# wbhart/mpir-fft

Measured on AMD Instinct MI355X. Metric: limbs/s for new_mpn_mul N×N-bit at 1/2/4/8 MI355X; % HBM roofline, higher is better.
Workload: dtype u64; 1 GPU; C3: new_mpn_mul depth=15 w=4 n1=n2=20312500 limbs (l=2048 limbs/coeff, NC x NR = 256 x 256, trunc=39936); parallelism=single

## Files before the change

__graft_entry__.py:

```python
import os
import subprocess
import sys

ROOT = os.path.dirname(os.path.abspath(__file__))
CSRC = os.path.join(ROOT, "mpir-fft_amd", "csrc")
LIB = os.path.join(ROOT, "mpir-fft_amd", "libmpfft.so")
HIPCC = os.environ.get("HIPCC", "/opt/rocm/bin/hipcc")


def build_lib(force=False):
    if force:
        subprocess.run(["make", "-s", "-C", CSRC, "clean"], check=True)
    jobs = str(min(8, os.cpu_count() or 1))
    subprocess.run(["make", "-s", "-C", CSRC, "-j" + jobs, "HIPCC=" + HIPCC], check=True)
    subprocess.run(["make", "-s", "-C", CSRC, "-j" + jobs, "HIPCC=" + HIPCC, "pwspill"], check=True)


def build_oracle():
    subprocess.run(["make", "-s", "-C", os.path.join(ROOT, "oracle")], check=True)


def build_c_caller():
    subprocess.run(["make", "-s", "-C", os.path.join(ROOT, "tests", "c_abi")], check=True)


def build_host_tests():
    subprocess.run(["make", "-s", "-C", os.path.join(ROOT, "tests", "pw_host")], check=True)


def build():
    build_lib()
    build_oracle()
    build_c_caller()
    build_host_tests()
    sys.path.insert(0, ROOT)
    import mpfft_loader
    m = mpfft_loader.load()
    assert m.lib().mpfft_version() >= 1


def smoke():
    import numpy as np
    import torch
    sys.path.insert(0, ROOT)
    sys.path.insert(0, os.path.join(ROOT, "oracle"))
    import mpfft_loader
    import oracle as O
    m = mpfft_loader.load()
    assert torch.cuda.is_available(), "smoke() needs a GPU"
    depth, w, n1, n2 = 9, 2, 120, 97
    a = m.fill_random(n1, 0x1001)
    b = m.fill_random(n2, 0x2002)
    dev = torch.device("cuda:0")
    da = torch.from_numpy(a.view(np.int64)).to(dev)
    db = torch.from_numpy(b.view(np.int64)).to(dev)
    dr = torch.zeros(n1 + n2, dtype=torch.int64, device=dev)
    ws = m.alloc_workspace(n1, n2, depth, w, dev)
    m.mul_device(dr, da, n1, db, n2, depth, w, ws)
    torch.cuda.synchronize()
    got = dr.cpu().numpy().view(np.uint64)
    want = O.new_mpn_mul(a, b, depth, w)
    assert (got == want).all(), "GPU new_mpn_mul differs from the oracle"
    assert O.to_int(got) == O.to_int(a) * O.to_int(b), "GPU product is not the exact product"
    r = np.zeros(n1 + n2, dtype=np.uint64)
    m.new_mpn_mul(r, a, n1, b, n2, depth, w)
    assert (r == want).all()
    d6, w6, m1, m2 = 8, 1, 700, 500
    a6 = m.fill_random(m1, 0x61)
    b6 = m.fill_random(m2, 0x62)
    r6 = m.mul6(a6, b6, d6, w6)
    assert (r6 == O.new_mpn_mul6(a6, b6, d6, w6)).all(), "GPU new_mpn_mul6 differs from the oracle"
    assert O.to_int(r6) == O.to_int(a6) * O.to_int(b6)
    print("smoke: ok (depth=%d w=%d n1=%d n2=%d; mul6 depth=%d w=%d n1=%d n2=%d)" % (depth, w, n1, n2, d6, w6, m1, m2))


if __name__ == "__main__":
    build()
    if len(sys.argv) > 1 and sys.argv[1] == "smoke":
        smoke()
```

mpir-fft_amd/csrc/kernels.hpp:

```cpp
#pragma once
#include "coeff.hpp"

struct PassArgs {
    u64 *dig[2];
    u64 *cb[2];
    int *top[2];
    const u64 *src[2];
    long nsrc[2];
    long src_chunk;
    u64 bits1;
    u64 N;
    int l;
    int lbM, lvl0;
    u64 rho;
    long sub_stride, pos_stride;
    int nsub, pos_off;
    int pbb;
    long pbs;
    int sub_off;
    long jNC;
    int zero_from;
    int need;
    int need_lo;
    int tw_mode;
    u64 tw_w;
    int tw_lbR;
    int canon;
    int ngroups;
    int nbuf;
    u64 scale_e;
    int ablate;
    unsigned *zp;
    long zn;
    unsigned long long *dbg;
    int pcarry;
    int pkeep;
    int fill_lo, fill_off;
    u64 fill_rho;
    int fill_hmin;
    int grp0;
};

__device__ inline void pass_clear_flags(const PassArgs &a)
{
    if (!a.zp) return;
    const long nt = (long)blockDim.x * blockDim.y * blockDim.z;
    const long nthr = (long)gridDim.x * gridDim.y * gridDim.z * nt;
    const long bid = ((long)blockIdx.z * gridDim.y + blockIdx.y) * gridDim.x + blockIdx.x;
    const long t = bid * nt + ((long)threadIdx.z * blockDim.y + threadIdx.y) * blockDim.x + threadIdx.x;
    for (long i = t; i < a.zn; i += nthr) a.zp[i] = 0u;
}

struct Lds {
    i64 *stage;
    int *edge;
    u64 *scr;
};

__host__ __device__ inline size_t lds_bytes(int l, int rb, int G, int U, int nw)
{
    size_t st = (size_t)rb * 2 * l * sizeof(i64);
    size_t ed = ((size_t)norm_edge_ints(G, U, nw) * sizeof(int) + 15) / 16 * 16;
    return st + ed + (size_t)norm_scr_u64(G, U, nw) * sizeof(u64);
}

template <int U, int G>
__device__ __forceinline__ Lds lds_carve(unsigned char *smem, int l, int rb, int nw)
{
    Lds d;
    d.stage = (i64 *)smem;
    unsigned char *p = smem + (size_t)rb * 2 * l * sizeof(i64);
    d.edge = (int *)p;
    p += ((size_t)norm_edge_ints(G, U, nw) * sizeof(int) + 15) / 16 * 16;
    d.scr = (u64 *)p;
    return d;
}

template <int U, int G, typename EF>
__device__ __forceinline__ void rotate_all(const WG &c, i64 (&x)[G][2 * U], EF efn, u64 N, int l, i64 *stage,
                                           int rb)
{
    if (U == 1 || rb >= G) {
        bool any = false;
#pragma unroll
        for (int i = 0; i < G; ++i) {
            const u64 e = efn(i);
            if (e) {
                rot_write<U>(c, x[i], stage + (size_t)i * 2 * l, l);
                any = true;
            }
        }
        if (!any) return;
        __syncthreads();
#pragma unroll
        for (int i = 0; i < G; ++i) {
            const u64 e = efn(i);
            if (e) rot_read<U>(c, x[i], stage + (size_t)i * 2 * l, make_rot(e, N), l);
        }
        __syncthreads();
    } else if (U != 1) {
#pragma unroll
        for (int i = 0; i < G; ++i) {
            const u64 e = efn(i);
            if (!e) continue;
// ... 967 lines not shown
```

mpir-fft_amd/csrc/mpfft.hip:

```cpp
#include <hip/hip_runtime.h>
#include <stdint.h>
#include <stdio.h>
#include <stdlib.h>
#include <string.h>
#include <mutex>
#include <string>
#include <vector>

#include "kernels.hpp"
#include "combine.hpp"
#include "fold.hpp"
#include "wdispatch.hpp"
#include "bdispatch.hpp"
#include "pdispatch.hpp"
#include "rdispatch.hpp"
#include "../../include/mpfft.h"

static const char *diag_env(const char *name)
{
#ifdef MPFFT_DIAG
    return getenv(name);
#else
    (void)name;
    return nullptr;
// ... 551 lines not shown
        HIPCHK(hipMemcpyAsync(h, d, nwg * 64, hipMemcpyDeviceToHost, s));
        HIPCHK(hipStreamSynchronize(s));
        double sum[8] = {0};
        long cnt = 0;
        unsigned long long t0 = ~0ull, t1 = 0;
        for (size_t w = 0; w < nwg; ++w) {
            const unsigned long long *q = h + 8 * w;
            if (!q[7]) continue;
            ++cnt;
            if (q[0] < t0) t0 = q[0];
            if (q[7] > t1) t1 = q[7];
            unsigned long long prev = q[0];
            for (int k = 1; k < 8; ++k)
                if (q[k]) { sum[k] += (double)(q[k] - prev); prev = q[k]; }
        }
        fprintf(stderr, "%s logg=%d dir=%d l=%ld groups=%ld/%zu span=%llu ticks: load %.0f lv0 %.0f lv1 %.0f lv2 %.0f fin %.0f canon/hx %.0f store %.0f\n", nthr == RP_NT || nthr == 1024 ? "rp_stamps" : "bp_stamps",
                logg, dir, P.l, cnt, nwg, t1 - t0, sum[1] / cnt, sum[2] / cnt, sum[3] / cnt, sum[4] / cnt, sum[5] / cnt,
                sum[6] / cnt, sum[7] / cnt);
        free(h);
        (void)hipFree(d);
        return MPFFT_OK;
    }

    PassArgs base_args(const View &v) const
    {
        PassArgs a;
        memset(&a, 0, sizeof(a));
        for (int k = 0; k < 2; ++k) {
            a.dig[k] = v.dig[k];
            a.cb[k] = v.cb[k];
            a.top[k] = v.top[k];
        }
        a.bits1 = P.bits1;
        a.N = P.N;
        a.l = (int)P.l;
        a.pbb = 30;
        a.jNC = P.NC;
        return a;
    }

    PassArgs col_args() const
    {
        PassArgs a = base_args(col);
        a.sub_stride = 1;
        a.pos_stride = ccount;
        a.nsub = ccount;
        a.sub_off = c0;
        return a;
    }

    PassArgs row_args() const
    {
        PassArgs a = base_args(row);
        a.lbM = P.lbC;
        a.rho = (u64)P.w * P.NR;
        a.sub_stride = ccb;
        a.pos_stride = 1;
        a.pbb = cbb;
        a.pbs = cbs;
        a.nsub = rcount;
        a.sub_off = r0;
        a.zero_from = (int)P.NC;
        a.need = (int)P.NC;
        a.tw_w = (u64)P.w;
        a.tw_lbR = P.lbR;
        return a;
    }

    static PassArgs only(PassArgs a, int op)
    {
        if (op == 1) {
            a.dig[0] = a.dig[1];
            a.cb[0] = a.cb[1];
            a.top[0] = a.top[1];
            a.src[0] = a.src[1];
            a.nsrc[0] = a.nsrc[1];
        }
        return a;
    }

    PassArgs col_pass_args(int lvl) const
    {
        PassArgs a = col_args();
        a.zero_from = (int)P.NR;
        a.lbM = P.lbR;
        a.lvl0 = lvl;
        a.rho = (u64)P.w * P.NC;
        a.need = (int)P.Tr;
        if (own_hi > 0) {
            a.need = own_hi < a.need ? own_hi : a.need;
            a.need_lo = own_lo;
        }
        return a;
    }

    int fwd_columns(const u64 *srcA, long nA, const u64 *srcB, long nB, int nops, int op = -1)
    {
        int lvl = 0, pend0 = 0;
        while (lvl < P.lbR) {
            PassArgs a = col_pass_args(lvl);
            if (lvl == 0) {
                a.src[0] = srcA; a.nsrc[0] = nA;
                a.src[1] = srcB; a.nsrc[1] = nB;
                a.src_chunk = src_chunk;
                a.zero_from = in_rows ? in_rows : (int)P.Tr;
                a.zp = zflags;
                a.zn = zflags_n;
            }
            if (op == 1) a.zp = nullptr;
            a.pcarry = lvl - pend0;
            const int k = fit(split(P.lbR - lvl, true), 0, [&](int) { return a; });
            if (carry_pend && rp_mode(a, k, 0) >= 0 && (carry_mask() & 1) && lvl + k < P.lbR) {
                const int k2 = split(P.lbR - lvl - k, true);
                PassArgs n = col_pass_args(lvl + k);
                n.pcarry = k;
                a.pkeep = rp_mode(n, k2, 0) >= 0;
            }
            int rc = op < 0 ? pass(a, k, 0, nops) : pass(only(a, op), k, 0, 1);
            if (rc) return rc;
            pend0 = a.pkeep ? lvl : lvl + k;
            lvl += k;
        }
        return MPFFT_OK;
    }

    int row_fused() const
    {
        static const bool off = [] { const char *e = diag_env("MPFFT_FUSE_ROW"); return e && !strcmp(e, "0"); }();
        const int f = P.fuse_rows;
        return fuse_row_last && !off && f && cview.dig[0] && pw_pair_kernel(P.l, f) && ccb >= (1 << f) ? f : 0;
    }

    int row_levels() const { return P.lbC - row_fused(); }

    PassArgs row_pass_args(int lvl, int k, int L) const
    {
        PassArgs a = row_args();
        a.lvl0 = lvl;
        a.tw_mode = lvl == 0 ? 1 : 0;
        if (lvl + k == L) a.canon = pwss_active() ? 0 : 1;
        return a;
    }

    int fwd_rows(int nops, int op = -1)
    {
        int lvl = 0, pend0 = 0;
        const int L = row_levels();
        while (lvl < L) {
            auto mk = [&](int kk) {
                PassArgs b = row_pass_args(lvl, kk, L);
                b.pcarry = lvl - pend0;
                return b;
            };
            const int k = fit(split(L - lvl), 0, mk);
            PassArgs a = mk(k);
            if (carry_pend && (carry_mask() & 4) && lvl + k < L && rp_mode(a, k, 0) >= 0) {
                const int k2 = split(L - lvl - k);
                PassArgs n = row_pass_args(lvl + k, k2, L);
                n.pcarry = k;
                a.pkeep = rp_mode(n, k2, 0) >= 0;
            }
            int rc = op < 0 ? pass(a, k, 0, nops) : pass(only(a, op), k, 0, 1);
            if (rc) return rc;
            pend0 = a.pkeep ? lvl : lvl + k;
            lvl += k;
        }
        return MPFFT_OK;
    }

  public:
    static int pwss_lk(long l) { return pwss_lk_of(l); }

    bool pwss_active() const
    {
        const int lk = pwss_lk(P.l);
        return lk && pw_get(pw_inner_limbs(P.l, lk), lk) != nullptr;
    }

    long pw_count = 0;

    int pointwise()
    {
        const long cnt = pw_count > 0 ? pw_count : (long)rcount * P.NC;
        if (cnt == 0) return MPFFT_OK;
        if (const int lk = pwss_lk(P.l)) {
            const int M = pw_inner_limbs(P.l, lk);
            const int fz = row_fused();
            const bool pair = fz > 0;
// ... 584 lines not shown
    if ((rc = X1.pointwise())) return rc;
    if (two && (rc = X2.pointwise())) return rc;
    pc.mark(3, s);
    if (fused) {
        XS.col = XS.row = X1.col;
        XC.col = XC.row = X1.col;
    }
    if ((rc = X1.inv_rows())) return rc;
    if (two && (rc = X2.inv_rows())) return rc;
    pc.mark(4, s);
    if ((rc = X1.itft(0, P.NR, P.NR))) return rc;
    if (two) {
        if ((rc = s2_launch(P, X1, S2_FILL, nullptr, nullptr, P2.Tr * P.NC, (P.NR - P2.Tr) * P.NC, 0, 1))) return rc;
        if ((rc = X2.itft1(0, P.NR, P2.Tr))) return rc;
    }
    if ((rc = s2_launch(P, X1, S2_IBFLY, nullptr, nullptr, 0, 2 * P.n, tlo > 0 ? tlo : 0, 1))) return rc;
    pc.mark(5, s);
    if ((rc = XS.scale())) return rc;
    pc.mark(6, s);
    rc = XC.combine_single(d_r, ws);
    pc.mark(7, s);
    return rc;
}

struct HostB {
    const u64 *h;
    hipStream_t cs;
    hipEvent_t ready;
};

static int run_all(const Plan &P, u64 *d_r, const u64 *d_i1, const u64 *d_i2, unsigned char *ws, hipStream_t s,
                   const HostB *hb = nullptr)
{
    if (P.sqrt2) return run_all6(P, d_r, d_i1, d_i2, ws, s);
    Exec X(P, s);
    X.single(ws);
    X.zflags = X.comb_flags(ws);
    X.zflags_n = X.comb_flag_words(P, P.total);
    X.drive_single();
    X.fuse_row_last = true;
    ProfCall pc;
    int rc;
    pc.mark(0, s);
    if (hb && hb->h) {
        if ((rc = X.fwd_columns(d_i1, P.n1, d_i2, P.n2, 1, 0))) return rc;
        if ((rc = X.fwd_rows(1, 0))) return rc;
        HIPCHK(hipMemcpyAsync((void *)d_i2, hb->h, (size_t)P.n2 * 8, hipMemcpyHostToDevice, hb->cs));
        HIPCHK(hipEventRecord(hb->ready, hb->cs));
        HIPCHK(hipStreamWaitEvent(s, hb->ready, 0));
        if ((rc = X.fwd_columns(d_i1, P.n1, d_i2, P.n2, 1, 1))) return rc;
        if ((rc = X.fwd_rows(1, 1))) return rc;
        pc.mark(1, s);
    } else {
        if ((rc = X.fwd_columns(d_i1, P.n1, d_i2, P.n2, 2))) return rc;
        pc.mark(1, s);
        if ((rc = X.fwd_rows(2))) return rc;
    }
    pc.mark(2, s);
    if ((rc = X.pointwise())) return rc;
    pc.mark(3, s);
    if ((rc = X.inv_rows())) return rc;
    pc.mark(4, s);
    if ((rc = X.itft(0, P.NR, P.Tr))) return rc;
    pc.mark(5, s);
    if ((rc = X.scale())) return rc;
    pc.mark(6, s);
    rc = X.fold ? X.combine_fold(d_r, ws, X.dbl_lo, X.dbl_hi) : X.combine_single(d_r, ws);
    pc.mark(7, s);
    return rc;
}

static std::string inv_columns_launches(const Plan &P)
{
    std::string out;
    if (P.sqrt2) return out;
    Exec X(P, nullptr);
    X.single(nullptr);
    X.drive_single();
    X.rec = &out;
    if (X.itft(0, P.NR, P.Tr)) out.clear();
    return out;
}

extern "C" {

int mpfft_inv_columns_schedule(long n1, long n2, unsigned long depth, unsigned long w, char *buf, size_t len)
{
    Plan P;
    int rc = make_plan(&P, n1, n2, depth, w);
    if (rc) return rc;
    const std::string s = inv_columns_launches(P);
    if (!buf || s.size() + 1 > len) return MPFFT_EINVAL;
    memcpy(buf, s.c_str(), s.size() + 1);
    return MPFFT_OK;
}

int mpfft_stage_kernels(long n1, long n2, unsigned long depth, unsigned long w, char *buf, size_t len)
{
    Plan P;
    int rc = make_plan(&P, n1, n2, depth, w);
    if (rc) return rc;
    const char *pass = P.big ? (P.rpass ? "k_rpass" : "k_bpass") : (P.wave && P.lds) ? "k_lpass" : P.wave ? "k_wpass" : "k_pass";
    char pw[96];
    const int lk = Exec::pwss_lk(P.l);
    const char *rows = P.big && P.rpass && !(lk && pw_get(pw_inner_limbs(P.l, lk), lk)) ? "k_rpass + k_bpass (canonical last pass)" : pass;
    const char *fz = diag_env("MPFFT_FUSE_ROW");
    const bool fused = P.has_c && !(fz && !strcmp(fz, "0"));
    if (lk && pw_get(pw_inner_limbs(P.l, lk), lk))
        snprintf(pw, sizeof pw, "k_pwss<%d>%s (nested negacyclic, K=%d)", pw_inner_limbs(P.l, lk),
                 !fused ? "" : P.fuse_rows == 2 ? " quad + last two row levels" : " pair + last row level", 1 << lk);
    else if (P.l % 256 == 0 && P.l <= 4096 && pw_kind() != PW_MFMA1 && pw_kind() != PW_VALU)
        snprintf(pw, sizeof pw, "k_pwm2 (int8 MFMA)");
    else if (P.l % 128 == 0 && pw_kind() != PW_VALU)
        snprintf(pw, sizeof pw, "k_pwm (int8 MFMA)");
    else if (P.l % 2 == 0 && P.l >= 32)
        snprintf(pw, sizeof pw, "k_pw (VALU)");
    else
        snprintf(pw, sizeof pw, "k_pointwise (VALU)");
    const char *pair = P.rpass ? "k_rpair" : P.wave ? "k_wpair" : "k_pairop";
    const char *scale = P.fuse_scale ? "(fused into the last inverse column pass)"
                        : P.fold ? "(folded: 2^-(depth+1) in the last inverse row pass)"
                        : P.rpass ? "k_rscale" : P.wave ? "k_wscale" : "k_scale";
    const char *comb = P.fold ? "k_cmeta + k_combine_red (reduced form)" : "k_combine1";
    char invc[96];
    int d1 = 0, d0 = 0;
    const std::string sched = inv_columns_launches(P);
    const size_t ha = sched.find(" halfadd ");
    if (ha != std::string::npos && sscanf(sched.c_str() + ha, " halfadd %d..%d", &d1, &d0) == 2)
        snprintf(invc, sizeof invc, "%s (FILL + half-add d=%d..%d) + %s", pass, d1, d0, pair);
    else
        snprintf(invc, sizeof invc, "%s + %s", pass, pair);
    snprintf(buf, len, "%s;%s;%s;%s;%s;%s;%s", pass, rows, pw, pass, invc, scale, comb);
    return MPFFT_OK;
}

int mpfft_profile_begin(int max_calls)
{
    std::lock_guard<std::mutex> lk(g_prof_mu);
    if (max_calls < 1 || g_prof.inflight > 0) return MPFFT_EINVAL;
    const int per = MPFFT_NSTAGES + 1;
    if (g_prof.cap < max_calls) {
        for (int i = 0; i < g_prof.cap * per; ++i) (void)hipEventDestroy(g_prof.ev[i]);
        free(g_prof.ev);
        free(g_prof.marks);
        g_prof.cap = 0;
        g_prof.ev = (hipEvent_t *)calloc((size_t)max_calls * per, sizeof(hipEvent_t));
        g_prof.marks = (int *)calloc((size_t)max_calls, sizeof(int));
        if (!g_prof.ev || !g_prof.marks) return MPFFT_ENOMEM;
        for (int i = 0; i < max_calls * per; ++i)
            if (hipEventCreate(&g_prof.ev[i]) != hipSuccess) {
                for (int j = 0; j < i; ++j) (void)hipEventDestroy(g_prof.ev[j]);
                return MPFFT_EHIP;
            }
        g_prof.cap = max_calls;
    }
    for (int c = 0; c < g_prof.cap; ++c) g_prof.marks[c] = 0;
    g_prof.used = 0;
    g_prof.on = true;
    return MPFFT_OK;
}

int mpfft_profile_end(float *stage_ms, int *calls)
{
    std::lock_guard<std::mutex> lk(g_prof_mu);
    g_prof.on = false;
    for (int k = 0; k < MPFFT_NSTAGES; ++k) stage_ms[k] = 0.f;
    int done = 0;
    for (int c = 0; c < g_prof.used; ++c) {
        if (g_prof.marks[c] != MPFFT_NSTAGES + 1) continue;
        hipEvent_t *e = g_prof.ev + (size_t)c * (MPFFT_NSTAGES + 1);
        if (hipEventSynchronize(e[MPFFT_NSTAGES]) != hipSuccess) return MPFFT_EHIP;
        for (int k = 0; k < MPFFT_NSTAGES; ++k) {
            float ms = 0.f;
            if (hipEventElapsedTime(&ms, e[k], e[k + 1]) != hipSuccess) return MPFFT_EHIP;
            stage_ms[k] += ms;
        }
        ++done;
    }
    if (calls) *calls = done;
    return MPFFT_OK;
}

const char *mpfft_strerror(int code)
{
    switch (code) {
    case MPFFT_OK: return "ok";
    case MPFFT_EINVAL: return "invalid parameters (need n1,n2 >= 1, 2 <= depth <= 30, n*w % 64 == 0)";
    case MPFFT_ETOOBIG: return "operands too large for the convolution: need j1 + j2 - 1 <= 2^(depth+1)";
    case MPFFT_EUNSUPPORTED: return "coefficient size n*w/64 > 4096 limbs is not supported";
    case MPFFT_ENOMEM: return "device allocation failed";
    case MPFFT_EHIP: return hipGetErrorString(last_hip_error);
    case MPFFT_ENODEV: return "no HIP device";
    }
    return "unknown error";
}

int mpfft_version(void) { return MPFFT_VERSION; }

int mpfft_check_params(long n1, long n2, unsigned long depth, unsigned long w)
{
    Plan P;
    return make_plan(&P, n1, n2, depth, w);
}

size_t mpfft_workspace_bytes(long n1, long n2, unsigned long depth, unsigned long w)
{
    Plan P;
    if (make_plan(&P, n1, n2, depth, w)) return 0;
    return P.bytes;
}

int mpfft_workspace_layout(long n1, long n2, unsigned long depth, unsigned long w, size_t *out)
{
    Plan P;
    int rc = make_plan(&P, n1, n2, depth, w);
// ... 430 lines not shown
```

mpir-fft_amd/csrc/rdispatch.hpp:

```cpp
#pragma once
#include <stddef.h>
#include <stdint.h>

struct PassArgs;
struct PairArgs;
typedef void (*rp_fn)(PassArgs);
typedef void (*rp_pair_fn)(PairArgs);

#define RP_NT 512

#ifdef MPFFT_FWD1K
#define RP_FWD1K 1
#else
#define RP_FWD1K 0
#endif
constexpr int rp_nt(int l, int logg, int dir = 0)
{
    return (l == 4096 && logg == 3) || (l == 2048 && logg == 4) || (l == 2048 && logg == 3 && (dir == 1 || RP_FWD1K)) ? 1024 : RP_NT;
}
constexpr int rp_r(int PP, int NT) { return 512 * PP / NT; }

rp_fn rp_get(int l, int logg, int dir, int mode);

inline int rp_maxlogg(int l) { return l == 1024 ? 3 : l == 2048 ? 3 : l == 4096 ? 3 : 0; }
inline int rp_maxlogg_fwd4(int l) { return l == 2048 ? 4 : rp_maxlogg(l); }
inline int rp_maxlogg_dit(int l) { return l == 2048 ? 4 : rp_maxlogg(l); }

inline size_t rp_lds(int l, int logg)
{
    const int G = 1 << logg, NX = G / 2 > 2 ? G / 2 : 2;
    const int nt = rp_nt(l, logg, 0), R = 512 * (l / 1024) / nt;
    return (size_t)NX * 9 * l + 4 * (size_t)(3 * G + (G / 2) * logg)
           + 20 * (size_t)(nt / 64) * G * R;
}

rp_pair_fn rp_pair_get(int l, int op);
inline size_t rp_pair_lds(int l) { return (size_t)9 * l + 16; }

rp_pair_fn rp_chain_get(int l, int nb);
inline size_t rp_chain_lds(int l) { return (size_t)9 * l + 32; }

typedef void (*rp_scale_fn)(uint64_t *, uint64_t *, int *, unsigned, unsigned, unsigned, unsigned, unsigned);
rp_scale_fn rp_scale_get(int l, int nt = 512);
inline size_t rp_scale_lds(int l) { return (size_t)9 * l + (size_t)l + 128; }
```

mpir-fft_amd/csrc/rkernels.hpp:

```cpp
#pragma once
#include "bkernels.hpp"
#include "rdispatch.hpp"

typedef unsigned long long rp_v2u __attribute__((ext_vector_type(2)));

#define RP_FENCE() do { asm volatile("" ::: "memory"); __builtin_amdgcn_sched_barrier(0); } while (0)

__device__ __forceinline__ u32 rp_uniform(u32 v) { return (u32)__builtin_amdgcn_readfirstlane((int)v); }

__device__ __forceinline__ int rp_launder(int t)
{
    asm volatile("" : "+v"(t));
    return t;
}

typedef unsigned int rp_v4u __attribute__((ext_vector_type(4)));

struct Pr {
    u32 w[4];
    int h;
};

__device__ __forceinline__ Pr pr_make(rp_v4u v, int h)
{
// ... 97 lines not shown
    i64 seq[6];
    bool swr[3];
#pragma unroll
    for (int k = 0; k < 3; ++k) {
        int m = m0 + k;
        const bool wr = m < 0;
        m += wr ? l : 0;
        const u64 f = F[m];
        i64 lo = (i64)(u32)f;
        if (!((m0 + k) & 1)) {
            const i64 hv = H[m ? (m >> 1) - 1 : l / 2 - 1];
            lo += m ? hv : -hv;
        }
        seq[2 * k] = lo;
        seq[2 * k + 1] = (i64)(f >> 32);
        swr[k] = wr;
    }
    i64 o[4];
#pragma unroll
    for (int k = 0; k < 4; ++k) {
        const i64 d1 = odd ? seq[k + 2] : seq[k + 1], d0 = odd ? seq[k + 1] : seq[k];
        const bool w1 = odd ? swr[(k + 2) >> 1] : swr[(k + 1) >> 1], w0 = odd ? swr[(k + 1) >> 1] : swr[k >> 1];
        o[k] = bp_cneg(bp_lo(d1, sb), w1) + bp_cneg(bp_hi(d0, sb), w0);
    }
    if (sg) {
#pragma unroll
        for (int k = 0; k < 4; ++k) o[k] = -o[k];
    }
    const i128 t0 = (i128)o[0] + ((i128)o[1] << 32);
    const i128 t1 = (i128)o[2] + ((i128)o[3] << 32) + (t0 >> 64);
    Pr r;
    r.w[0] = (u32)t0;
    r.w[1] = (u32)((u64)t0 >> 32);
    r.w[2] = (u32)t1;
    r.w[3] = (u32)((u64)t1 >> 32);
    r.h = (int)(i64)(t1 >> 64);
    return r;
}

__device__ __forceinline__ u32 rp_fun(u32 hi, u32 lo, u32 s) { return s ? __builtin_amdgcn_alignbit(hi, lo, 32 - s) : hi; }

template <int B>
__device__ __forceinline__ Pr rp_shift_pair(const Pr &a, const Pr &b, u32 s, bool sub)
{
    const u32 bs = b.h < 0 ? ~0u : 0u;
    auto aw = [&](int i) -> u32 { return i >= 0 && i < 4 ? a.w[i] : 0u; };
    auto bw = [&](int i) -> u32 { return i < 4 ? b.w[i] : i == 4 ? (u32)b.h : bs; };
    Pr lo, hi;
#pragma unroll
    for (int k = 0; k < 4; ++k) {
        lo.w[k] = rp_fun(aw(k - B), aw(k - B - 1), s);
        hi.w[k] = rp_fun(bw(k + 4 - B), bw(k + 3 - B), s);
    }
    lo.h = 0;
    hi.h = (int)rp_fun(bw(8 - B), bw(7 - B), s);
    const u32 m = sub ? ~0u : 0u;
    return pr_addx(lo, hi, m, (u32)sub);
}

template <int PP>
__device__ __forceinline__ Pr rp_get_rot(const RX<PP> &X, int j, int pp, u32 e, u32 N)
{
    constexpr int HP = RX<PP>::l / 2;
    const u32 d = e & 127;
    bool n0, n1;
    const Pr a = pr_cneg(rp_get_al<PP>(X, j, pp, e - d, N, n0), n0);
    if (d == 0) return a;
    const Pr b = pr_cneg(rp_get_al<PP>(X, j, pp ? pp - 1 : HP - 1, e - d, N, n1), n1);
    const u32 s = d & 31;
    const bool wrap = pp == 0;
    switch (d >> 5) {
    case 0: return rp_shift_pair<0>(a, b, s, wrap);
    case 1: return rp_shift_pair<1>(a, b, s, wrap);
    case 2: return rp_shift_pair<2>(a, b, s, wrap);
    default: return rp_shift_pair<3>(a, b, s, wrap);
    }
}

#ifndef RP_GX_LOAD
#define RP_GX_LOAD 1
#endif
#ifndef RP_SPLIT_ZSKIP
#define RP_SPLIT_ZSKIP 1
#endif
#ifndef RP_SPLIT_LDS
#define RP_SPLIT_LDS 1
#endif
#ifndef RP_SPLIT_PROBE
#define RP_SPLIT_PROBE 0
#endif
__device__ __forceinline__ u32 rp_ror1(u32 v) { return (u32)__builtin_amdgcn_update_dpp(0, (int)v, 0x13C, 0xF, 0xF, false); }

template <int G, int PP, int NT, typename EF>
__device__ __forceinline__ void rp_shift_all(Pr (&x)[G][rp_r(PP, NT)], u32 *EDGE, EF ef, int t)
{
    constexpr int R = rp_r(PP, NT), NW = NT / 64;
    const int lane = t & 63, wv = t >> 6;
    if (lane == 63) {
#pragma unroll
        for (int i = 0; i < G; ++i)
#pragma unroll
            for (int r = 0; r < R; ++r) {
                u32 *q = EDGE + 5 * ((wv * G + i) * R + r);
                q[0] = x[i][r].w[0];
                q[1] = x[i][r].w[1];
                q[2] = x[i][r].w[2];
                q[3] = x[i][r].w[3];
                q[4] = (u32)x[i][r].h;
            }
    }
    __syncthreads();
#pragma unroll
    for (int i = 0; i < G; ++i) {
        const u32 d = ef(i) & 127;
        if (d == 0) continue;
        const u32 s = d & 31;
#pragma unroll
        for (int r = 0; r < R; ++r) {
            RP_FENCE();
            Pr b;
            b.w[0] = rp_ror1(x[i][r].w[0]);
            b.w[1] = rp_ror1(x[i][r].w[1]);
            b.w[2] = rp_ror1(x[i][r].w[2]);
            b.w[3] = rp_ror1(x[i][r].w[3]);
            b.h = (int)rp_ror1((u32)x[i][r].h);
            if (lane == 0) {
                const int w2 = wv ? wv - 1 : NW - 1, r2 = wv ? r : (r ? r - 1 : R - 1);
                const u32 *q = EDGE + 5 * ((w2 * G + i) * R + r2);
                b.w[0] = q[0];
                b.w[1] = q[1];
                b.w[2] = q[2];
                b.w[3] = q[3];
                b.h = (int)q[4];
            }
            const bool wrap = t == 0 && r == 0;
            switch (d >> 5) {
            case 0: x[i][r] = rp_shift_pair<0>(x[i][r], b, s, wrap); break;
            case 1: x[i][r] = rp_shift_pair<1>(x[i][r], b, s, wrap); break;
            case 2: x[i][r] = rp_shift_pair<2>(x[i][r], b, s, wrap); break;
            default: x[i][r] = rp_shift_pair<3>(x[i][r], b, s, wrap); break;
            }
        }
    }
}

__device__ __forceinline__ u32 rp_mod2n(u32 e, u32 N2)
{
    e = e >= 2 * N2 ? e - 2 * N2 : e;
    return e >= N2 ? e - N2 : e;
}

template <int LOGG, int DIR>
__device__ __forceinline__ u32 rp_tw(const PassArgs &a, const BGeo &g, int li, int k)
{
    const int JB = DIR == 0 ? LOGG - 1 - li : li;
    const int level = DIR == 0 ? a.lvl0 + li : a.lvl0 + LOGG - 1 - li;
    const u32 h = 1u << (a.lbM - level - 1);
    const u32 unit = (u32)a.rho << level;
    return (u32)(g.pos0 & (h - 1)) * unit + (u32)(k & ((1 << JB) - 1)) * (u32)g.pstep * unit;
}

__device__ __forceinline__ u32 rp_pend_pos(u32 rho, int lbM, int lo, int hi, u32 p, u32 N2)
{
    const u32 xm = p & ((1u << (lbM - hi)) - 1);
    u32 e = 0;
    for (int lev = lo; lev < hi; ++lev)
// ... 234 lines not shown
    constexpr int l = 1024 * PP, HP = l / 2, cbw = 2 * l / 64, R = rp_r(PP, NT);
    t = rp_launder(t);
#pragma unroll
    for (int i = 0; i < NS; ++i)
#pragma unroll
        for (int r = 0; r < R; ++r) HX[i * HP + t + NT * r] = (short)x[i][r].h;
    __syncthreads();
    const int lane = t & 63, wv = t >> 6;
#pragma unroll
    for (int i = 0; i < NS; ++i) {
        if (!keep(i)) continue;
        const long sl = (long)rp_uniform(SL[i]);
        u64 *dst = st.dig + (size_t)sl * l;
        u64 *cbp = st.cb + (size_t)sl * cbw;
#pragma unroll
        for (int r = 0; r < R; ++r) {
            RP_FENCE();
            const int pp = t + NT * r;
            const int hv = HX[i * HP + (pp ? pp - 1 : HP - 1)];
            const int hin = pp ? hv : -hv;
            int k0;
            u32 w0 = x[i][r].w[0], w1 = x[i][r].w[1];
            add_small(w0, w1, hin, k0);
            *(rp_v4u *)(dst + 2 * pp) = rp_v4u{w0, w1, x[i][r].w[2], x[i][r].w[3]};
            const u64 bp = __ballot(k0 == 1), bn = __ballot(k0 == -1);
            const u64 pa = rp_spread32((u32)bp), na = rp_spread32((u32)bn);
            const u64 pb = rp_spread32((u32)(bp >> 32)), nb = rp_spread32((u32)(bn >> 32));
            if (lane < 2)
                *(rp_v2u *)(cbp + 2 * (2 * (wv + (NT / 64) * r) + lane)) = lane ? rp_v2u{pb, nb} : rp_v2u{pa, na};
        }
        if (t == 0) st.top[sl] = 0;
    }
}

template <int G, int R>
__device__ __forceinline__ void rp_pin(Pr (&x)[G][R])
{
#pragma unroll
    for (int i = 0; i < G; ++i)
#pragma unroll
        for (int r = 0; r < R; ++r)
            asm volatile("" : "+v"(x[i][r].w[0]), "+v"(x[i][r].w[1]), "+v"(x[i][r].w[2]), "+v"(x[i][r].w[3]), "+v"(x[i][r].h));
    RP_FENCE();
}

template <int LOGG, int PP, int DIR, int MODE>
__global__ __launch_bounds__(rp_nt(1024 * PP, LOGG, DIR), 4) void k_rpass(PassArgs a)
{
    constexpr int NT = rp_nt(1024 * PP, LOGG, DIR), R = rp_r(PP, NT);
    constexpr bool GX = DIR == 0 ? MODE == 1 : (MODE & 1) != 0, SPLIT = DIR == 0 && MODE == 2,
                   CIN = DIR == 0 && MODE == 3, HL = DIR == 1 && (MODE & 2) != 0,
                   FILL = DIR == 1 && (MODE & 4) != 0, LTW = DIR == 1 && (MODE & 8) != 0;
    pass_clear_flags(a);
    constexpr int G = 1 << LOGG, NX = G / 2 > 2 ? G / 2 : 2;
    constexpr int l = 1024 * PP, HP = l / 2, cbw = 2 * l / 64;
    extern __shared__ __attribute__((aligned(16))) unsigned char smem[];
    const RX<PP> X{smem};
    const int t = threadIdx.x;
    const u32 N = (u32)a.N, N2 = 2 * (u32)a.N;
    const int op = blockIdx.y;
    Coef st;
    st.dig = a.dig[op];
    st.cb = a.cb[op];
    st.top = a.top[op];
    const int sub = __builtin_amdgcn_readfirstlane((int)(blockIdx.x / a.ngroups));
    const int grp = __builtin_amdgcn_readfirstlane((int)(a.grp0 + blockIdx.x % a.ngroups));
    const int lobits = a.lbM - a.lvl0 - LOGG;
    const int lo = grp & ((1 << lobits) - 1);
    const int hi = grp >> lobits;
    const int bstart = hi << (a.lbM - a.lvl0);
    if (DIR == 0 && (bstart >= a.need || bstart + (1 << (a.lbM - a.lvl0)) <= a.need_lo)) return;
    BGeo g;
    g.pos0 = bstart | lo;
    g.pstep = 1 << lobits;
    g.sbase = (long)sub * a.sub_stride;
    const u64 rsub = a.tw_mode && a.tw_mode != 3 ? (u64)revbin_dev(a.sub_off + sub, a.tw_lbR) : 0;
    g.tw0 = a.tw_mode == 3 ? a.tw_w * (u64)(a.sub_off + sub) : a.tw_w * (u64)(a.pos_off + g.pos0) * rsub;
    g.twst = a.tw_w * (u64)g.pstep * rsub;
    auto slot_lane = [&](int i) -> long {
        const int ps = a.pos_off + g.pos0 + i * g.pstep;
        return g.sbase + (long)(ps >> a.pbb) * a.pbs + (long)(ps & ((1 << a.pbb) - 1)) * a.pos_stride;
    };
    auto slot_of = [&](int i) -> long { return wv_uniform(slot_lane(i)); };
    auto zero_in = [&](int i) -> bool { return SPLIT && g.pos0 + i * g.pstep >= a.zero_from; };
    constexpr int NEXP = 2 * G + (G / 2) * LOGG;
    u32 *EXPT = (u32 *)(smem + NX * RX<PP>::SB);
    u32 *SLT = EXPT + NEXP;
    if (t < NEXP) EXPT[t] = rp_exp_entry<LOGG, DIR, GX, CIN>(a, g, t, N2, 0u);
    else if (t < NEXP + G) SLT[t - NEXP] = (u32)slot_lane(t - NEXP);
    __syncthreads();
    const u64 *src = SPLIT ? a.src[op] : nullptr;
    unsigned long long *stamp = a.dbg ? a.dbg + 8 * ((size_t)blockIdx.y * gridDim.x + blockIdx.x) : nullptr;
#define RP_STAMP(k) do { if (stamp && t == 0) stamp[k] = __builtin_amdgcn_s_memtime(); } while (0)
    RP_STAMP(0);

    unsigned short *CODE = (unsigned short *)smem;
    Pr x[G][R];
    u32 *EDGE = SLT + G;
    if ((DIR == 0 && GX && RP_GX_LOAD) || LTW) {
        auto ef = [&](int i) -> u32 { return rp_uniform(EXPT[i]); };
        const RpCodes cd = rp_codes_load<G, PP>(st, SLT, t);
        rp_load_limbs_rot<G, G, PP, NT>(x, st, SLT, ef, t);
        rp_codes_store<G, PP>(CODE, cd, t);
        __syncthreads();
        rp_decode_rot<G, G, PP, NT>(x, CODE, ef, t);
        rp_pin<G, R>(x);
        rp_shift_all<G, PP, NT>(x, EDGE, ef, t);
    } else if (CIN) {
        auto ef = [&](int i) -> u32 { return rp_uniform(EXPT[i]); };
        const RpCodes cd = rp_codes_load<G, PP>(st, SLT, t);
        rp_load_limbs_rot<G, G, PP, NT>(x, st, SLT, ef, t);
        rp_codes_store<G, PP>(CODE, cd, t);
        __syncthreads();
        rp_decode_rot<G, G, PP, NT>(x, CODE, ef, t);
        rp_pin<G, R>(x);
    } else if (!SPLIT) {
        const RpCodes cd = rp_codes_load<G, PP>(st, SLT, t);
        rp_load_limbs<G, G, PP, NT>(x, st, SLT, t);
        rp_codes_store<G, PP>(CODE, cd, t);
        __syncthreads();
        rp_decode<G, G, PP, NT>(x, CODE, t);
    } else {
        auto split_pair = [](u64 x0, u64 x1, u64 x2, int sh, u64 left) -> Pr {
            u64 f0 = sh ? (x0 >> sh) | (x1 << (64 - sh)) : x0;
            u64 f1 = sh ? (x1 >> sh) | (x2 << (64 - sh)) : x1;
            f0 = left < 64 ? f0 & ((((u64)1) << left) - 1) : f0;
            f1 = left <= 64 ? 0 : left < 128 ? f1 & ((((u64)1) << (left - 64)) - 1) : f1;
            return pr_make(rp_v4u{(u32)f0, (u32)(f0 >> 32), (u32)f1, (u32)(f1 >> 32)}, 0);
        };
        constexpr int SWP = l / 4 + 2, SW = 2 * SWP, KR = (G * SWP + NT - 1) / NT;
        constexpr bool STAGE = RP_SPLIT_LDS && (size_t)G * SW * 8 <= (size_t)NX * RX<PP>::SB;
        if (STAGE && !a.src_chunk) {
            u64 *S = (u64 *)smem;
            const long nsv = a.nsrc[op];
            auto slot_q0 = [&](int i) -> long {
                const long j = (long)(a.pos_off + g.pos0 + i * g.pstep) * a.jNC + a.sub_off + sub;
                return (long)(((u64)j * a.bits1) >> 6) & ~1L;
            };
            rp_v4u v[KR];
#pragma unroll
            for (int k = 0; k < KR; ++k) {
                const int idx = t + NT * k, i = idx / SWP, u = idx - i * SWP;
                v[k] = rp_v4u{0, 0, 0, 0};
                if (i < G && !zero_in(i)) {
                    const long q = slot_q0(i) + 2 * u;
                    if (q + 1 < nsv) {
                        v[k] = *(const rp_v4u *)(src + q);
                    } else if (q < nsv) {
                        const u64 w = src[q];
                        v[k] = rp_v4u{(u32)w, (u32)(w >> 32), 0, 0};
                    }
                }
            }
#pragma unroll
            for (int k = 0; k < KR; ++k) {
                const int idx = t + NT * k, i = idx / SWP, u = idx - i * SWP;
                if (i < G && !zero_in(i)) *(rp_v4u *)(S + (long)i * SW + 2 * u) = v[k];
            }
            __syncthreads();
#pragma unroll
            for (int i = 0; i < G; ++i) {
                const bool z = zero_in(i);
                const long j = (long)(a.pos_off + g.pos0 + i * g.pstep) * a.jNC + a.sub_off + sub;
                const long qa = (long)(((u64)j * a.bits1) >> 6) & ~1L;
#pragma unroll
                for (int r = 0; r < R; ++r) {
                    const int pp = t + NT * r;
                    x[i][r] = Pr{{0, 0, 0, 0}, 0};
                    const u64 left = (u64)pp * 128 < a.bits1 ? a.bits1 - (u64)pp * 128 : 0;
                    if (z || !left) continue;
                    const u64 off = (u64)j * a.bits1 + (u64)pp * 128;
                    const u64 *sp = S + (long)i * SW + ((long)(off >> 6) - qa);
                    x[i][r] = split_pair(sp[0], sp[1], sp[2], (int)(off & 63), left);
                }
            }
            __syncthreads();
        } else {
#pragma unroll
            for (int i = 0; i < G; ++i) {
                __builtin_amdgcn_sched_barrier(0);
                const bool z = zero_in(i);
#pragma unroll
                for (int r = 0; r < R; ++r) {
                    const int pp = t + NT * r;
                    x[i][r] = Pr{{0, 0, 0, 0}, 0};
                    if (z) continue;
                    const u64 left = (u64)pp * 128 < a.bits1 ? a.bits1 - (u64)pp * 128 : 0;
                    const long j = (long)(a.pos_off + g.pos0 + i * g.pstep) * a.jNC + a.sub_off + sub;
                    const u64 off = (u64)j * a.bits1 + (u64)pp * 128;
                    const long q = (long)(off >> 6);
                    const long ns = left ? a.nsrc[op] : 0;
                    const SrcSlice sv{a.src_chunk, a.jNC, a.sub_off};
#if RP_SPLIT_PROBE
                    const u64 x0 = left ? (u64)q * 0x9e3779b97f4a7c15ull : 0, x1 = x0 ^ (u64)j, x2 = x1 + 1;
#else
                    const u64 x0 = src_limb(src, ns, sv, j, a.bits1, q), x1 = src_limb(src, ns, sv, j, a.bits1, q + 1),
                              x2 = src_limb(src, ns, sv, j, a.bits1, q + 2);
#endif
                    x[i][r] = split_pair(x0, x1, x2, (int)(off & 63), left);
                }
            }
        }
    }
    RP_STAMP(1);
    if (DIR == 0 && GX && !RP_GX_LOAD) {
        rp_rot_all<G, PP, NX, NT>(x, X, [&](int s) -> u32 { return rp_uniform(EXPT[s]); }, N, t);
    }

#pragma unroll
    for (int li = 0; li < LOGG; ++li) {
        const int JB = DIR == 0 ? LOGG - 1 - li : li;
        if ((DIR == 0 && li == 0) || (DIR == 1 && li == 0 && HL)) {
#pragma unroll
            for (int pi = 0; pi < G / 2; ++pi) {
                const int i = ((pi >> JB) << (JB + 1)) | (pi & ((1 << JB) - 1));
                const int k = i | (1 << JB);
#pragma unroll
                for (int r = 0; r < R; ++r) {
                    const Pr y = x[k][r];
                    pr_bfly(x[i][r], x[k][r], x[i][r], y, false);
                }
            }
            if (li < 3) RP_STAMP(2 + li);
            continue;
        }
        auto pz = [&](int k) -> bool { return RP_SPLIT_ZSKIP && SPLIT && zero_in(k & ((1 << (LOGG - li)) - 1)); };
        const int tl = rp_launder(t);
        bool xch = false;
#pragma unroll
        for (int pi = 0; pi < G / 2; ++pi) {
            const int i = ((pi >> JB) << (JB + 1)) | (pi & ((1 << JB) - 1));
            if (pz(i | (1 << JB))) continue;
            rp_pub<PP, NT>(X, pi, x[i | (1 << JB)], tl);
            xch = true;
        }
        if (xch) __syncthreads();
#pragma unroll
        for (int pi = 0; pi < G / 2; ++pi) {
            const int i = ((pi >> JB) << (JB + 1)) | (pi & ((1 << JB) - 1));
            const int k = i | (1 << JB);
            if (pz(k)) {
#pragma unroll
                for (int r = 0; r < R; ++r) x[k][r] = x[i][r];
                continue;
            }
            const u32 E = rp_uniform(EXPT[2 * G + (G / 2) * li + pi]);
#pragma unroll
            for (int r = 0; r < R; ++r) {
                if (r % 2 == 0) RP_FENCE();
                bool ng;
                const Pr y = rp_get_al<PP>(X, pi, tl + NT * r, E, N, ng);
                pr_bfly(x[i][r], x[k][r], x[i][r], y, ng);
            }
        }
        if (xch) __syncthreads();
        if (li < 3) RP_STAMP(2 + li);
    }
    if (DIR == 0 && !a.pkeep && a.lvl0 + LOGG < a.lbM) {
        rp_rot_all_al<G, PP, NX, NT>(x, X, [&](int s) -> u32 { return rp_uniform(EXPT[G + s]); }, N, t);
    }
    if (DIR == 1) rp_pin<G, R>(x);
    if (DIR == 1 && GX) {
        rp_rot_all<G, PP, NX, NT>(x, X, [&](int s) -> u32 { return rp_uniform(EXPT[s]); }, N, t);
    }
    RP_STAMP(5);

    if (DIR == 1) rp_pin<G, R>(x);
    rp_store<G, G, PP, NT>(x, st, SLT, [&](int i) -> bool {
        const int bs = (g.pos0 + i * g.pstep) & ~(g.pstep - 1);
        return DIR == 1 || (bs < a.need && bs + g.pstep > a.need_lo);
    }, (short *)smem, t);
    if (FILL) {
        if (t < G) {
            const int p = g.pos0 + t * g.pstep;
            u32 e = 0, keep = 0;
            if (p >= a.fill_lo) {
                int q = p, c = 0;
                for (int d = a.fill_off >> 1; a.fill_hmin && d >= a.fill_hmin; d >>= 1) {
                    if (q >= a.fill_lo + d && q < 2 * d) {
                        q -= d;
                        ++c;
                    } else if (q < d) {
                        ++c;
                    }
                }
                e = rp_mod2n((u32)(((u64)p * a.fill_rho) % N2) + N2 - (u32)c, N2);
                keep = q == p;
            }
            EXPT[t] = e;
            EXPT[G + t] = keep;
        }
        __syncthreads();
        if (t < G) SLT[t] += (u32)((long)a.fill_off * a.pos_stride);
        constexpr bool FPIN = PP == 4 && LOGG == 3;
        if (FPIN) rp_pin<G, R>(x);
        rp_rot_all<G, PP, NX, NT, true>(x, X, [&](int s) -> u32 { return rp_uniform(EXPT[s]); }, N, t);
        if (FPIN) rp_pin<G, R>(x);
        if (a.fill_hmin) {
#pragma unroll
            for (int dl = LOGG - 1; dl >= 0; --dl) {
                const int ds = 1 << dl;
                if (ds * g.pstep < a.fill_hmin) continue;
#pragma unroll
                for (int s = 0; s < ds; ++s) {
                    if (g.pos0 + s * g.pstep < a.fill_lo) continue;
#pragma unroll
                    for (int r = 0; r < R; ++r) x[s][r] = pr_add(x[s][r], x[s + ds][r]);
                }
            }
            if (FPIN) rp_pin<G, R>(x);
        }
        rp_store<G, G, PP, NT>(x, st, SLT, [&](int s) -> bool { return rp_uniform(EXPT[G + s]) != 0; }, (short *)smem, t);
    }
    RP_STAMP(6);
    if (stamp) {
        __syncthreads();
        RP_STAMP(7);
    }
#undef RP_STAMP
}

template <int PP, int OP>
__global__ __launch_bounds__(RP_NT) void k_rpair(PairArgs a)
{
    constexpr int l = 1024 * PP;
    constexpr bool LOADB = OP != OP_DOUBLE && OP != OP_FILL;
    extern __shared__ __attribute__((aligned(16))) unsigned char smem[];
    const RX<PP> X{smem};
    u32 *SL = (u32 *)(smem + RX<PP>::SB);
    const int t = threadIdx.x;
    const int col = (int)(blockIdx.x % a.ncol);
    const int i = a.i0 + (int)(blockIdx.x / a.ncol);
    const u32 N = (u32)a.N, N2 = 2 * (u32)a.N;
    const u32 e = (u32)(((u64)i * a.rho) % N2);
// ... 283 lines not shown
```

Before: 5.520 billion limbs/s.

## Prune zero-input butterflies per operand in split forward column pass

Computes a per-operand zero-row boundary from each input's actual length, so the first forward column pass skips butterflies and LDS publishes for slots known to be zero. It adds a level-0 copy path for zero partners and, where a butterfly class has only one live input, publishes that value once and reuses it across the class. This is meant to cut VALU and LDS exchange work when the inputs are truncated, at the cost of extra index logic and a wider per-operand zero description. It also adds a schedule-reporting helper and a host test build.

```diff
diff --git a/__graft_entry__.py b/__graft_entry__.py
--- a/__graft_entry__.py
+++ b/__graft_entry__.py
@@ -26,6 +26,7 @@
 
 def build_host_tests():
     subprocess.run(["make", "-s", "-C", os.path.join(ROOT, "tests", "pw_host")], check=True)
+    subprocess.run(["make", "-s", "-C", os.path.join(ROOT, "tests", "split_prune_host")], check=True)
 
 
 def build():
diff --git a/mpir-fft_amd/csrc/kernels.hpp b/mpir-fft_amd/csrc/kernels.hpp
--- a/mpir-fft_amd/csrc/kernels.hpp
+++ b/mpir-fft_amd/csrc/kernels.hpp
@@ -20,6 +20,7 @@
     int sub_off;
     long jNC;
     int zero_from;
+    int zero_op[2];
     int need;
     int need_lo;
     int tw_mode;
diff --git a/mpir-fft_amd/csrc/mpfft.hip b/mpir-fft_amd/csrc/mpfft.hip
--- a/mpir-fft_amd/csrc/mpfft.hip
+++ b/mpir-fft_amd/csrc/mpfft.hip
@@ -657,7 +657,7 @@
     PassArgs col_pass_args(int lvl) const
     {
         PassArgs a = col_args();
-        a.zero_from = (int)P.NR;
+        a.zero_from = a.zero_op[0] = a.zero_op[1] = (int)P.NR;
         a.lbM = P.lbR;
         a.lvl0 = lvl;
         a.rho = (u64)P.w * P.NC;
@@ -679,6 +679,13 @@
                 a.src[1] = srcB; a.nsrc[1] = nB;
                 a.src_chunk = src_chunk;
                 a.zero_from = in_rows ? in_rows : (int)P.Tr;
+                a.zero_op[0] = a.zero_op[1] = a.zero_from;
+                if (srcA && srcB && !src_chunk && !in_rows) {
+                    a.zero_op[0] = (int)rp_zero_row(P.j1, P.NC, P.Tr);
+                    a.zero_op[1] = (int)rp_zero_row(P.j2, P.NC, P.Tr);
+                    if (op >= 0) a.zero_op[0] = a.zero_op[1] = a.zero_op[op];
+                    a.zero_from = std::max(a.zero_op[0], a.zero_op[1]);
+                }
                 a.zp = zflags;
                 a.zn = zflags_n;
             }
@@ -1429,6 +1436,19 @@
     return out;
 }
 
+static std::string fwd_columns_launches(const Plan &P)
+{
+    std::string out;
+    if (P.sqrt2) return out;
+    static const u64 none = 0;
+    Exec X(P, nullptr);
+    X.single(nullptr);
+    X.drive_single();
+    X.rec = &out;
+    if (X.fwd_columns(&none, P.n1, &none, P.n2, 2)) out.clear();
+    return out;
+}
+
 extern "C" {
 
 int mpfft_inv_columns_schedule(long n1, long n2, unsigned long depth, unsigned long w, char *buf, size_t len)
@@ -1477,7 +1497,13 @@
         snprintf(invc, sizeof invc, "%s (FILL + half-add d=%d..%d) + %s", pass, d1, d0, pair);
     else
         snprintf(invc, sizeof invc, "%s + %s", pass, pair);
-    snprintf(buf, len, "%s;%s;%s;%s;%s;%s;%s", pass, rows, pw, pass, invc, scale, comb);
+    char fwdc[64];
+    int fg = 0, fp = 0, fn = 0;
+    if (sscanf(fwd_columns_launches(P).c_str(), "k_rpass<%d,%d,0,2>%n", &fg, &fp, &fn) == 2 && fn > 0)
+        snprintf(fwdc, sizeof fwdc, "%s (split: k_rpass<%d,%d,0,2>)", pass, fg, fp);
+    else
+        snprintf(fwdc, sizeof fwdc, "%s", pass);
+    snprintf(buf, len, "%s;%s;%s;%s;%s;%s;%s", fwdc, rows, pw, pass, invc, scale, comb);
     return MPFFT_OK;
 }
 
diff --git a/mpir-fft_amd/csrc/rdispatch.hpp b/mpir-fft_amd/csrc/rdispatch.hpp
--- a/mpir-fft_amd/csrc/rdispatch.hpp
+++ b/mpir-fft_amd/csrc/rdispatch.hpp
@@ -26,6 +26,35 @@
 inline int rp_maxlogg_fwd4(int l) { return l == 2048 ? 4 : rp_maxlogg(l); }
 inline int rp_maxlogg_dit(int l) { return l == 2048 ? 4 : rp_maxlogg(l); }
 
+#ifdef __HIPCC__
+#define RP_HD __host__ __device__
+#else
+#define RP_HD
+#endif
+RP_HD inline long rp_zero_row(long j, long NC, long cap)
+{
+    const long z = (j + NC - 1) / NC;
+    return z < cap ? z : cap;
+}
+RP_HD inline int rp_live_slots(int G, int pos0, int lstep, int zf)
+{
+    if (zf <= pos0) return 0;
+    const int n = (int)(((long)zf - pos0 + (1L << lstep) - 1) >> lstep);
+    return n < G ? n : G;
+}
+RP_HD inline int rp_pair_of(int logg, int li, int k)
+{
+    const int jb = logg - 1 - li;
+    return ((k >> (jb + 1)) << jb) | (k & ((1 << jb) - 1));
+}
+RP_HD inline bool rp_class_single(int logg, int li, int nlive, int k, int &rep)
+{
+    const int m = 1 << (logg - li), c = k & (m - 1);
+    const bool single = c < nlive && c + m >= nlive;
+    rep = single ? c : k;
+    return single;
+}
+
 inline size_t rp_lds(int l, int logg)
 {
     const int G = 1 << logg, NX = G / 2 > 2 ? G / 2 : 2;
diff --git a/mpir-fft_amd/csrc/rkernels.hpp b/mpir-fft_amd/csrc/rkernels.hpp
--- a/mpir-fft_amd/csrc/rkernels.hpp
+++ b/mpir-fft_amd/csrc/rkernels.hpp
@@ -203,6 +203,12 @@
 #endif
 #ifndef RP_SPLIT_ZSKIP
 #define RP_SPLIT_ZSKIP 1
+#endif
+#ifndef RP_SPLIT_L0COPY
+#define RP_SPLIT_L0COPY 1
+#endif
+#ifndef RP_SPLIT_PUB1
+#define RP_SPLIT_PUB1 1
 #endif
 #ifndef RP_SPLIT_LDS
 #define RP_SPLIT_LDS 1
@@ -603,7 +609,8 @@
         return g.sbase + (long)(ps >> a.pbb) * a.pbs + (long)(ps & ((1 << a.pbb) - 1)) * a.pos_stride;
     };
     auto slot_of = [&](int i) -> long { return wv_uniform(slot_lane(i)); };
-    auto zero_in = [&](int i) -> bool { return SPLIT && g.pos0 + i * g.pstep >= a.zero_from; };
+    const int nlive = SPLIT ? __builtin_amdgcn_readfirstlane(rp_live_slots(G, g.pos0, lobits, a.zero_op[op])) : G;
+    auto zero_in = [&](int i) -> bool { return SPLIT && i >= nlive; };
     constexpr int NEXP = 2 * G + (G / 2) * LOGG;
     u32 *EXPT = (u32 *)(smem + NX * RX<PP>::SB);
     u32 *SLT = EXPT + NEXP;
@@ -736,6 +743,12 @@
             for (int pi = 0; pi < G / 2; ++pi) {
                 const int i = ((pi >> JB) << (JB + 1)) | (pi & ((1 << JB) - 1));
                 const int k = i | (1 << JB);
+                constexpr bool L0COPY = RP_SPLIT_ZSKIP && RP_SPLIT_L0COPY && SPLIT && !(PP == 4 && LOGG == 2);
+                if (L0COPY && zero_in(k)) {
+#pragma unroll
+                    for (int r = 0; r < R; ++r) x[k][r] = x[i][r];
+                    continue;
+                }
 #pragma unroll
                 for (int r = 0; r < R; ++r) {
                     const Pr y = x[k][r];
@@ -746,12 +759,17 @@
             continue;
         }
         auto pz = [&](int k) -> bool { return RP_SPLIT_ZSKIP && SPLIT && zero_in(k & ((1 << (LOGG - li)) - 1)); };
+        auto xs = [&](int pi, int k) -> int {
+            int rep = k;
+            if (RP_SPLIT_ZSKIP && RP_SPLIT_PUB1 && SPLIT && rp_class_single(LOGG, li, nlive, k, rep)) return rp_pair_of(LOGG, li, rep);
+            return pi;
+        };
         const int tl = rp_launder(t);
         bool xch = false;
 #pragma unroll
         for (int pi = 0; pi < G / 2; ++pi) {
             const int i = ((pi >> JB) << (JB + 1)) | (pi & ((1 << JB) - 1));
-            if (pz(i | (1 << JB))) continue;
+            if (pz(i | (1 << JB)) || xs(pi, i | (1 << JB)) != pi) continue;
             rp_pub<PP, NT>(X, pi, x[i | (1 << JB)], tl);
             xch = true;
         }
@@ -766,11 +784,12 @@
                 continue;
             }
             const u32 E = rp_uniform(EXPT[2 * G + (G / 2) * li + pi]);
+            const int xp = xs(pi, k);
 #pragma unroll
             for (int r = 0; r < R; ++r) {
                 if (r % 2 == 0) RP_FENCE();
                 bool ng;
-                const Pr y = rp_get_al<PP>(X, pi, tl + NT * r, E, N, ng);
+                const Pr y = rp_get_al<PP>(X, xp, tl + NT * r, E, N, ng);
                 pr_bfly(x[i][r], x[k][r], x[i][r], y, ng);
             }
         }
```

Result: faster. 5.621 billion limbs/s, median of 6 (+1.8%).
